# YuvalNirkin/hyperseg

Hardware: AMD Instinct MI355X
Metric: frames/sec @ bs=1 HyperSeg-M 1024x512 (higher is better)
Workload: dtype f32 storage and accumulation; level-4 inverted residual products as 3-term f16 splits (f32-class: 1.3e-7 of sum|a||b|; exact_f32 beside it)

## Files before the change

### hyperseg_amd/_hip.py

```python
import ctypes as C
import os
import types

import torch

_LIB_PATH = os.environ.get('HS_HIP_LIB') or os.path.join(os.path.dirname(os.path.abspath(__file__)), 'lib',
                                                         'libhyperseg_hip.so')

ACT_NONE, ACT_RELU, ACT_RELU6, ACT_SWISH = 0, 1, 2, 3
PAD_MODES = {'zeros': 0, 'reflect': 1, 'replicate': 2, 'circular': 3}
PREV_NONE, PREV_SAME, PREV_BILINEAR = 0, 1, 2

_STATUS = {-1: 'bad argument', -2: 'feature map does not tile into the weight grid (H % fh or W % fw != 0)',
           -3: 'unsupported shape', -4: 'tile does not fit the LDS'}


class HipLibraryError(RuntimeError):
    pass


class StageInputC(C.Structure):
    _fields_ = [('skip', C.c_void_p), ('prev', C.c_void_p),
                ('batch', C.c_int32), ('H', C.c_int32), ('W', C.c_int32),
                ('c_skip', C.c_int32), ('c_prev', C.c_int32),
# ... 167 lines not shown
    'hs_label_resize_batch_coded_fwd': ([vp, i32, i32, i32, i32, vp, vp, vp, i32, i32, i32, vp, i32, i32, i32, vp, i32, vp], STATUS),
    'hs_color_jitter_fwd': ([vp, i32, i32, i32, i32, vp, vp, vp, vp, vp], STATUS),
    'hs_gaussian_blur_fwd': ([vp, i32, i32, i32, i32, vp, vp, vp, vp, vp, vp], STATUS),
    'hs_frame_rotate_fwd': ([vp, i32, i32, i32, i32, vp, i32, i32, C.c_uint32, C.c_uint32, vp, vp, vp], STATUS),
    'hs_label_rotate_fwd': ([vp, i32, i32, i32, i32, vp, i32, i32, i32, i32, vp, i32, vp], STATUS),
    'hs_resize_tables_ragged_fwd': ([vp, i32, i32, i32, i32, i32, i32, i32, vp, vp, vp, vp, vp], STATUS),
    'hs_color_jitter_ragged_fwd': ([vp, i32, i32, i32, i32, vp, vp, vp, vp, vp], STATUS),
    'hs_frame_resize_ragged_fwd': ([vp, i32, i32, i32, i32, vp, vp, vp, vp, i32, i32, i32, vp, vp], STATUS),
    'hs_label_resize_ragged_fwd': ([vp, i32, i32, i32, i32, vp, vp, vp, i32, i32, vp, vp], STATUS),
    'hs_frame_rotate_ragged_fwd': ([vp, i32, i32, i32, i32, vp, vp, vp, i32, i32, C.c_uint32, C.c_uint32, vp, vp, vp], STATUS),
    'hs_label_rotate_ragged_fwd': ([vp, i32, i32, i32, vp, vp, vp, i32, i32, i32, i32, vp, i32, vp], STATUS),
    'hs_mbconv_expand_dw_fwd': ([vp, i32, i32, i32, i32, vp, i32, vp, vp, vp, i32, i32, i32, i32, i32, i32, vp, vp, vp, vp, vp], STATUS),
    'hs_se_gate_fwd': ([vp, i32, i32, i32, C.c_float, vp, vp, i32, vp, vp, vp, vp, vp, i32, vp, vp, vp], STATUS),
    'hs_gemm_split_kp': ([i32], C.c_int),
    'hs_gemm_split_fwd': ([vp, vp, vp, vp, vp, i32, vp, vp, i32, i32, i32, i32, i32, vp], STATUS),
    'hs_gemm_split_conv2x2_fwd': ([vp, vp, vp, vp, i32, vp, vp, i32, i32, i32, i32, i32, i32, vp], STATUS),
    'hs_gemm_split_up2_fwd': ([vp, vp, vp, vp, i32, vp, i32, i32, i32, i32, i32, i32, vp], STATUS),
    'hs_depthwise_route': ([i32] * 11, C.c_int),
    'hs_mbconv_route': ([i32] * 11, C.c_int),
    'hs_stem_dw_route': ([i32] * 9, C.c_int),
    'hs_stem_route': ([i32] * 3, C.c_int),
    'hs_se_gate_route': ([i32] * 5, C.c_int),
    'hs_pointwise_route': ([i32] * 5, C.c_int),
    'hs_pooled_shift_fwd': ([vp, i32, C.c_float, vp, vp, vp, i32, i32, vp], STATUS),
}
EXPORTS = list(SIGNATURES)


def check(status, what):
    if status == 0:
# ... 73 lines not shown
```

### hyperseg_amd/build.py

```python
import os
import shutil
import subprocess
import sys

PKG = os.path.dirname(os.path.abspath(__file__))
REPO = os.path.dirname(PKG)
CSRC = os.path.join(PKG, 'csrc')
LIB_DIR = os.path.join(PKG, 'lib')
LIB_PATH = os.path.join(LIB_DIR, 'libhyperseg_hip.so')
SOURCES = ['hs_weights.hip', 'hs_patch_conv.hip', 'hs_patch_conv_gen.hip', 'hs_patch_conv_k1m.hip', 'hs_k1_chain.hip', 'hs_meta_conv.hip', 'hs_patch_ir.hip', 'hs_patch_ir_fused.hip', 'hs_patch_irc.hip', 'hs_patch_ir_px.hip', 'hs_patch_ir_d2.hip', 'hs_encoder.hip', 'hs_mbconv.hip', 'hs_mbconv_lean.hip', 'hs_gemm_split.hip', 'hs_patch_conv_bwd.hip', 'hs_patch_conv_train.hip', 'hs_train_aux.hip', 'hs_s2w_train.hip', 'hs_eval.hip', 'hs_tta_merge.hip', 'hs_ingest.hip', 'hs_overlay.hip', 'hs_confidence.hip', 'hs_resample.hip', 'hs_resample_batch.hip', 'hs_jitter.hip', 'hs_blur.hip', 'hs_validate.hip', 'hs_rotate.hip', 'hs_augment_ragged.hip', 'hs_label_codec.hip']
HEADERS = [os.path.join(CSRC, 'hs_common.h'), os.path.join(CSRC, 'hs_ir_tiles.h'), os.path.join(CSRC, 'hs_ir_common.h'), os.path.join(CSRC, 'hs_s2w_blocked.h'), os.path.join(CSRC, 'hs_se_tail.h'), os.path.join(CSRC, 'hs_upsample_taps.h'), os.path.join(CSRC, 'hs_ingest.h'), os.path.join(CSRC, 'hs_resample_px.h'), os.path.join(CSRC, 'hs_resample_tables.h'), os.path.join(CSRC, 'hs_jitter_px.h'), os.path.join(CSRC, 'hs_blur_px.h'), os.path.join(CSRC, 'hs_rotate_px.h'), os.path.join(CSRC, 'hs_eval_count.h'), os.path.join(CSRC, 'hs_last_launch.h'), os.path.join(CSRC, 'hs_confidence.h'), os.path.join(CSRC, 'hs_label_codec.h'), os.path.join(REPO, 'include', 'hyperseg_hip.h')]
FLAGS = ['--offload-arch=gfx950', '-O3', '-std=c++17', '-fPIC', '-ffp-contract=off', '-mllvm', '-amdgpu-kernarg-preload-count=16',
         '-Wall', '-Wno-unused-function', '-I', os.path.join(REPO, 'include'), '-I', CSRC]


def _hipcc():
    for cand in (os.environ.get('HIPCC'), shutil.which('hipcc'), '/opt/rocm/bin/hipcc'):
        if cand and os.path.exists(cand):
            return cand
    raise RuntimeError('hipcc not found (need ROCm >= 7.0 with gfx950 support)')


def needs_build():
    if not os.path.exists(LIB_PATH):
        return True
    t = os.path.getmtime(LIB_PATH)
# ... 36 lines not shown
```

### hyperseg_amd/csrc/hs_gemm_split.hip

```cpp
#include "hs_common.h"
#include <type_traits>

namespace hs {

using half8 = __attribute__((ext_vector_type(8))) _Float16;
using gs_f32x4 = __attribute__((ext_vector_type(4))) float;

__device__ __forceinline__ int gs_exp_of(float m) { return min(max(__float_as_int(m) >> 23, 27), 254); }
__device__ __forceinline__ float gs_scale_of(int eb) { return __int_as_float((268 - eb) << 23); }
__device__ __forceinline__ float gs_inv_scale_of(int eb) { return __int_as_float((eb - 14) << 23); }

struct GemmSplitArgs {
    const _Float16* __restrict__ wf;
    const float* __restrict__ w_inv;
    const float* __restrict__ gate; const float* __restrict__ x;
    const float* shift;
    const float* residual;
    float* y;
    int M, K, KST, N, act;
    int conv_wo;
    float* pool_partial;
    int up2_wo;
};

#ifndef HS_GS_NARROW_MAX_WG
#define HS_GS_NARROW_MAX_WG 128
#endif

#ifndef HS_GS_TALL_MIN_WG
#define HS_GS_TALL_MIN_WG 257
#endif

template <int KS, int NWV, bool FAST, int NS, int MT, int NCH, bool PATCH>
__global__ __launch_bounds__(64 * NWV)
void gemm_split_kernel(GemmSplitArgs a) {
    extern __shared__ __attribute__((aligned(16))) float gs_red[];
    constexpr int nthr = 64 * NWV, nwv = NWV;
    constexpr int NP = 16 * NS, NR = 16 * MT, NE = NR * NP;
    const int tid = threadIdx.x, lane = tid & 63, wave = tid >> 6;
    const int lrow = lane & 15, kg = lane >> 4;
    const int n0 = blockIdx.x * NP, r0 = blockIdx.y * MT, b = blockIdx.z;
    const float* __restrict__ xb = a.x + (size_t)b * a.K * a.N;
    const float* __restrict__ gb = a.gate ? a.gate + (size_t)b * a.K : nullptr;
    float* yb = a.y + (size_t)b * a.M * a.N * (a.up2_wo > 0 ? 4 : 1);
    const float* rb = a.residual ? a.residual + (size_t)b * a.M * a.N : nullptr;
    const int rt_max = (a.M + 15) >> 4;

    using gs_f32x2 = __attribute__((ext_vector_type(2))) float;
    const int ncol0 = min(n0 + NS * lrow, a.N - (FAST && !PATCH && NS == 2 ? 2 : 1)), ncol1 = min(n0 + NS * lrow + 1, a.N - 1);
    float xv[NCH][NS][KS][8];
// ... 33 lines not shown
                        const gs_f32x2 v = *reinterpret_cast<const gs_f32x2*>(xb + (size_t)kc * a.N + ncol0);
                        xv[c][0][s][j] = v[0]; xv[c][1][s][j] = v[1];
                    } else {
                        xv[c][0][s][j] = xb[(size_t)kc * a.N + ncol0]; xv[c][1][s][j] = xb[(size_t)kc * a.N + ncol1];
                    }
                }
    }
    constexpr int NG = PATCH ? 1 : NCH;
    float gv[NG][KS][8];
    if constexpr (!PATCH) {
#pragma unroll
        for (int c = 0; c < NCH; ++c)
#pragma unroll
            for (int s = 0; s < KS; ++s) {
                const int k0 = ((wave * NCH + c) * KS + s) * 32 + 8 * kg;
                if constexpr (FAST) {
                    const float* gp = gb ? gb + min(k0, a.K - 8) : a.w_inv;
                    const gs_f32x4 g0 = *reinterpret_cast<const gs_f32x4*>(gp), g1 = *reinterpret_cast<const gs_f32x4*>(gp + 4);
#pragma unroll
                    for (int j = 0; j < 4; ++j) { gv[c][s][j] = g0[j]; gv[c][s][4 + j] = g1[j]; }
                } else {
#pragma unroll
                    for (int j = 0; j < 8; ++j) gv[c][s][j] = gb ? gb[min(k0 + j, a.K - 1)] : 1.0f;
                }
            }
    }
    half8 ah[2][KS], al[2][KS];
    auto load_a = [&](int q) {
        const int rt = min(r0 + q % MT, rt_max - 1);
#pragma unroll
        for (int s = 0; s < KS; ++s) {
// ... 5 lines not shown
    load_a(0);
    constexpr int TE = (NE + nthr - 1) / nthr;
    float wi[TE], sh[TE], yo[TE];
    auto load_tail = [&]() {
#pragma unroll
        for (int i = 0; i < TE; ++i) {
            const int e = min(tid + i * nthr, NE - 1);
            const int row = min(16 * r0 + e / NP, a.M - 1), col = min(n0 + (e & (NP - 1)), a.N - 1);
            wi[i] = a.w_inv[min(16 * r0 + e / NP, 16 * rt_max - 1)];
            sh[i] = a.shift ? a.shift[row] : 0.0f;
            yo[i] = rb ? rb[(size_t)row * a.N + col] : 0.0f;
        }
    };
    constexpr bool LATE_TAIL = KS * NCH >= 3;
    if constexpr (!LATE_TAIL) load_tail();
    __builtin_amdgcn_sched_barrier(0);

    gs_f32x4 tot[MT][NS];
#pragma unroll
    for (int c = 0; c < NCH; ++c) {
        float invb[NS];
        half8 bh[NS][KS], bl[NS][KS];
#pragma unroll
        for (int t = 0; t < NS; ++t) {
            unsigned mx = 0;
#pragma unroll
            for (int s = 0; s < KS; ++s) {
                const int k0 = ((wave * NCH + c) * KS + s) * 32 + 8 * kg;
#pragma unroll
                for (int j = 0; j < 8; ++j) {
                    const float mk = (FAST || PATCH ? k0 : k0 + j) < a.K ? 1.0f : 0.0f;
                    float g = mk;
                    if constexpr (!PATCH) g = gb ? gv[c][s][j] * mk : mk;
                    xv[c][t][s][j] *= g;
                    mx = max(mx, __float_as_uint(xv[c][t][s][j]) & 0x7fffffffu);
                }
            }
            {
                auto r16 = __builtin_amdgcn_permlane16_swap(mx, mx, false, false);
                mx = max(r16[0], r16[1]);
                auto r32 = __builtin_amdgcn_permlane32_swap(mx, mx, false, false);
                mx = max(r32[0], r32[1]);
            }
            const int eb = gs_exp_of(__uint_as_float(mx));
            const float sc = gs_scale_of(eb);
            invb[t] = gs_inv_scale_of(eb);
#pragma unroll
            for (int s = 0; s < KS; ++s) {
// ... 128 lines not shown
    nch = per > 5 ? 2 : 1;
    ks = (steps + nwv * nch - 1) / (nwv * nch);
    return ks <= 5;
}

}

using namespace hs;

extern "C" int hs_gemm_split_kp(int32_t c_in) {
    int nwv, ks, nch;
    if (c_in <= 0 || !gemm_split_plan(c_in, nwv, ks, nch)) return HS_ERR_UNSUPPORTED;
    return nwv * nch * ks * 32;
}

static int launch_gemm_split_plain(const void* w_frag, const float* w_inv, const float* gate, const float* x, const float* shift,
                                   int32_t act, const float* residual, float* y, int32_t batch, int32_t c_out, int32_t c_in,
                                   int32_t kp, int32_t pixels, int up2_wo, void* stream) {
    if (!w_frag || !w_inv || !x || !y || batch <= 0 || c_out <= 0 || c_in <= 0 || pixels <= 0) return HS_ERR_BAD_ARG;
    if (act < 0 || act > 3) return HS_ERR_BAD_ARG;
    int nwv, ks, nch;
    if (!gemm_split_plan(c_in, nwv, ks, nch)) return HS_ERR_UNSUPPORTED;
    if (kp != nwv * nch * ks * 32 || (ks > 1 && nwv != 8)) return HS_ERR_BAD_ARG;
    if (batch > 65535 || (c_out + 31) / 32 > 65535) return HS_ERR_UNSUPPORTED;
    GemmSplitArgs a{(const _Float16*)w_frag, w_inv, gate, x, shift, residual, y, c_out, c_in, kp / 32, pixels, act, 0, nullptr, up2_wo};
    dim3 grid((pixels + 31) / 32, ((c_out + 15) / 16 + 1) / 2, batch);
    const size_t wgs = (size_t)grid.x * grid.y * grid.z;
    const bool narrow = wgs <= HS_GS_NARROW_MAX_WG && pixels > 16;
    const bool tall = wgs >= HS_GS_TALL_MIN_WG && c_out > 32;
    if (narrow) grid.x = (pixels + 15) / 16;
    if (tall) grid.y = ((c_out + 15) / 16 + 3) / 4;
    const size_t lds = (size_t)nwv * (narrow ? 512 : tall ? 2048 : 1024) * sizeof(float);
    hipStream_t s = (hipStream_t)stream;
    const bool fast = (c_in & 7) == 0 && (pixels & 1) == 0 && c_in >= 8;
#define HS_GS_(KSV, NWV, F) do { \
        if (narrow) hipLaunchKernelGGL((gemm_split_kernel<KSV, NWV, F, 1, 2, 1, false>), grid, dim3(64 * NWV), lds, s, a); \
        else if (tall) hipLaunchKernelGGL((gemm_split_kernel<KSV, NWV, F, 2, 4, 1, false>), grid, dim3(64 * NWV), lds, s, a); \
        else hipLaunchKernelGGL((gemm_split_kernel<KSV, NWV, F, 2, 2, 1, false>), grid, dim3(64 * NWV), lds, s, a); } while (0)
#define HS_GS(KSV, NWV) do { if (fast) HS_GS_(KSV, NWV, true); else HS_GS_(KSV, NWV, false); } while (0)
    if (nch == 2) {
        if (!fast || up2_wo > 0) return HS_ERR_UNSUPPORTED;
        grid.x = (pixels + 15) / 16; grid.y = ((c_out + 15) / 16 + 1) / 2;
        const size_t lds2 = (size_t)8 * 512 * sizeof(float);
#define HS_GS2(KSV) hipLaunchKernelGGL((gemm_split_kernel<KSV, 8, true, 1, 2, 2, false>), grid, dim3(512), lds2, s, a)
        switch (ks) { case 3: HS_GS2(3); break; case 4: HS_GS2(4); break; case 5: HS_GS2(5); break; default: return HS_ERR_UNSUPPORTED; }
#undef HS_GS2
        return launch_status();
    }
    switch (ks) {
        case 1: if (nwv == 2) HS_GS(1, 2); else if (nwv == 4) HS_GS(1, 4); else HS_GS(1, 8); break;
        case 2: HS_GS(2, 8); break;
        case 3: HS_GS(3, 8); break;
        case 4: HS_GS(4, 8); break;
        default: HS_GS(5, 8); break;
    }
#undef HS_GS
#undef HS_GS_
    return launch_status();
}

extern "C" int hs_gemm_split_fwd(const void* w_frag, const float* w_inv, const float* gate, const float* x,
                                 const float* shift, int32_t act, const float* residual, float* y,
                                 int32_t batch, int32_t c_out, int32_t c_in, int32_t kp, int32_t pixels, void* stream) {
    return launch_gemm_split_plain(w_frag, w_inv, gate, x, shift, act, residual, y, batch, c_out, c_in, kp, pixels, 0, stream);
}

extern "C" int hs_gemm_split_up2_fwd(const void* w_frag, const float* w_inv, const float* x, const float* shift, int32_t act,
                                     float* y, int32_t batch, int32_t c_out, int32_t c_in, int32_t kp, int32_t Ho, int32_t Wo,
                                     void* stream) {
    if (Ho <= 0 || Wo <= 0 || (((size_t)y) & 7) != 0) return HS_ERR_BAD_ARG;
    return launch_gemm_split_plain(w_frag, w_inv, nullptr, x, shift, act, nullptr, y, batch, c_out, c_in, kp, Ho * Wo, Wo, stream);
}
// ... 10 lines not shown
extern "C" int hs_gemm_split_conv2x2_fwd(const void* w_frag, const float* w_inv, const float* x, const float* shift, int32_t act,
                                         float* y, float* pool_partial, int32_t batch, int32_t c_out, int32_t c_in, int32_t kp,
                                         int32_t Ho, int32_t Wo, void* stream) {
    if (!w_frag || !w_inv || !x || !y || batch <= 0 || c_out <= 0 || c_in <= 0 || Ho <= 0 || Wo <= 0) return HS_ERR_BAD_ARG;
    if (act < 0 || act > 3) return HS_ERR_BAD_ARG;
    int nwv, ks, nch;
    if (c_in > (1 << 20) || !gemm_split_plan(4 * c_in, nwv, ks, nch) || nwv != 8 || (Wo & 1) || (c_in & 1)) return HS_ERR_UNSUPPORTED;
    if (kp != nwv * nch * ks * 32) return HS_ERR_BAD_ARG;
    if ((((size_t)x) & 15) != 0) return HS_ERR_BAD_ARG;
    const int pixels = Ho * Wo;
    if (batch > 65535 || (c_out + 31) / 32 > 65535) return HS_ERR_UNSUPPORTED;
    GemmSplitArgs a{(const _Float16*)w_frag, w_inv, nullptr, x, shift, nullptr, y, c_out, 4 * c_in, kp / 32, pixels, act, Wo, pool_partial, 0};
    dim3 grid((pixels + 15) / 16, ((c_out + 15) / 16 + 1) / 2, batch);
    const size_t lds = (size_t)8 * 512 * sizeof(float);
    hipStream_t s = (hipStream_t)stream;
#define HS_GP(KSV, NCHV) hipLaunchKernelGGL((gemm_split_kernel<KSV, 8, true, 1, 2, NCHV, true>), grid, dim3(512), lds, s, a)
    switch (ks * 2 + nch - 1) {
        case 2: HS_GP(1, 1); break;
        case 4: HS_GP(2, 1); break;
        case 6: HS_GP(3, 1); break;
        case 8: HS_GP(4, 1); break;
        case 10: HS_GP(5, 1); break;
        case 7: HS_GP(3, 2); break;
        case 9: HS_GP(4, 2); break;
        case 11: HS_GP(5, 2); break;
        default: return HS_ERR_UNSUPPORTED;
    }
#undef HS_GP
    return launch_status();
}
```

### hyperseg_amd/functional.py

```python
import collections
import ctypes as C
import functools
import os
import threading

import torch

from . import _hip
from ._hip import ACT_NONE, ACT_RELU, ACT_RELU6, PAD_MODES

BN_EPS_DEFAULT = 1e-5
DTYPE_CODES = {torch.float32: 0, torch.bfloat16: 1, torch.float16: 2}
S2W_TRAIN_MAX_LAYERS = 8
COSCHEDULE_BANKS = os.environ.get('HS_COSCHEDULE_BANKS', '0') == '1'


def _round_up(n, m):
    return (n + m - 1) // m * m


def _device_of(a):
    if isinstance(a, torch.Tensor):
        return a.device
    if isinstance(a, (StageInput, BankRef, SignalRef, U8Frame)):
# ... 1097 lines not shown
        raise ValueError(f'out has shape {tuple(out.shape)}, expected {shape}')
    if residual is not None and tuple(residual.shape) != shape:
        raise ValueError(f'residual has shape {tuple(residual.shape)}, expected {shape}')
    if gate is not None and tuple(gate.shape) != (b, cin):
        raise ValueError(f'gate has shape {tuple(gate.shape)}, expected {(b, cin)}')
    if shift is not None and shift.numel() != sw.c_out:
        raise ValueError(f'shift has {shift.numel()} entries, expected {sw.c_out}')
    _hip.run.hs_gemm_split_fwd(_hip.dev_ptr(sw.frag, 'w_frag', torch.float16), _hip.dev_ptr(sw.inv, 'w_inv'),
                               _hip.dev_ptr(gate, 'gate') if gate is not None else None, _hip.dev_ptr(x, 'x'),
                               _hip.dev_ptr(shift, 'shift') if shift is not None else None, int(act),
                               _hip.dev_ptr(residual, 'residual') if residual is not None else None,
                               _hip.dev_ptr(out, 'out'), b, sw.c_out, cin, sw.kp, h * w, _hip.stream_ptr())
    return out


@_on_operand_device
def gemm_split_conv2x2(sw, x, shift=None, act=ACT_NONE, out=None, pool_partial=None):
    b, cin, h, w = x.shape
    if 4 * cin != sw.c_in:
        raise ValueError(f'input has {cin} channels, the weight {sw.c_in} / 4')
    if h % 2 or w % 4:
        raise ValueError(f'map {h}x{w}: height must be even and width a multiple of 4')
    shape = (b, sw.c_out, h // 2, w // 2)
    if out is None:
        out = torch.empty(shape, device=x.device, dtype=torch.float32)
    elif tuple(out.shape) != shape:
        raise ValueError(f'out has shape {tuple(out.shape)}, expected {shape}')
    if shift is not None and shift.numel() != sw.c_out:
        raise ValueError(f'shift has {shift.numel()} entries, expected {sw.c_out}')
    nblk = -(-(h // 2) * (w // 2) // 16)
# ... 1018 lines not shown
```

### hyperseg_amd/utils/inference.py

```python
import contextlib
import os

import torch
import torch.nn as nn

from ..models._common import Blend, Epilogue, HyperGenBase, Score


class InputNorm:

    LAYOUTS = ('hwc', 'chw')

    def __init__(self, mean=(0.485, 0.456, 0.406), std=(0.229, 0.224, 0.225), layout='hwc'):
        if layout not in self.LAYOUTS:
            raise ValueError(f'layout {layout!r}: expected one of {self.LAYOUTS}')
        self.mean = torch.as_tensor(mean, dtype=torch.float32).flatten().clone()
        self.std = torch.as_tensor(std, dtype=torch.float32).flatten().clone()
        if self.mean.numel() != 3 or self.std.numel() != 3:
            raise ValueError('mean and std must hold one value per channel of a 3-channel frame')
        if bool((self.std == 0).any()):
            raise ValueError('std must be non-zero')
        self.layout = layout
        values = torch.arange(256, dtype=torch.float32)
        self._tables = {torch.device('cpu'): ((values.div(255)[None, :] - self.mean[:, None]) / self.std[:, None]).contiguous()}
# ... 179 lines not shown
            _fold(mods[i], mods[i + 1])
            seq[i + 1] = nn.Identity()
            n += 1
    return n


def _bn_affine(bn):
    with torch.no_grad():
        scale = bn.weight / torch.sqrt(bn.running_var + bn.eps)
        shift = bn.bias - bn.running_mean * scale
    return scale.detach().clone(), shift.detach().clone()


SPLIT_GEMM_MAX_K = int(os.environ.get('HS_SPLIT_GEMM_MAX_K', '1280'))
STEM_DW = os.environ.get('HS_STEM_DW', '1') != '0'
FUSE_EXPAND_MIN_PIXELS = int(os.environ.get('HS_FUSE_EXPAND_MIN_PIXELS', '2048'))
FUSE_EXPAND_MAX_CIN = int(os.environ.get('HS_FUSE_EXPAND_MAX_CIN', '40'))


LEAN_MFMA_MAX_CIN = int(os.environ.get('HS_LEAN_MFMA_MAX_CIN', '16'))
PW_MFMA_MAX_CIN = int(os.environ.get('HS_PW_MFMA_MAX_CIN', '96'))
PW_MFMA_MIN_PIXELS = int(os.environ.get('HS_PW_MFMA_MIN_PIXELS', '8192'))
GEMM_LT_MIN_PIXELS = int(os.environ.get('HS_GEMM_LT_MIN_PIXELS', '16384'))


@contextlib.contextmanager
def gemm_library(pixels, batch=1):
    want = os.environ.get('HS_BLAS') or ('cublaslt' if (pixels >= GEMM_LT_MIN_PIXELS or batch > 1) else 'cublas')
    prev = torch.backends.cuda.preferred_blas_library()
    torch.backends.cuda.preferred_blas_library(want)
# ... 185 lines not shown
                else:
                    x = self.expand(x)
            out = HF.depthwise_conv_bn_act(x, blk._depthwise_conv.weight, self.stride, self.pad_t, self.pad_l,
                                           (ho, wo), self.scale, self.shift, act=3, pool=True,
                                           in_scale=in_scale, in_shift=in_shift, se=se)
        y, pooled, gated = out if se is not None else (out[0], out[1], False)

        def se_gate(**fold):
            if gated and not fold:
                return pooled
            return HF.se_gate(pooled, b, ho * wo, red.weight, red.bias, self._exp_t, exp.bias, **fold)
        skip = inputs.contiguous() if self.skip else None
        if lean_gemm:
            sw = proj.split_weights(True, y.device) if proj.split_gemm else None
            if sw is not None:
                gate = se_gate()
                if self.defer_shift:
                    if skip is None:
                        return HF.gemm_split(sw, y, gate=gate)
                    return HF.gemm_split(sw, y, gate=gate, residual=skip, out=skip)
                return HF.gemm_split(sw, y, gate=gate, shift=proj.shift, residual=skip)
            wp = se_gate(w_proj=proj.conv.weight, out_scale=proj.scale)
            cmid = y.shape[1]
            with gemm_library(ho * wo, b):
                if b == 1:
                    w2d, y2d = wp.view(-1, cmid), y.view(cmid, ho * wo)
                    if self.defer_shift:
                        if skip is None:
                            return torch.mm(w2d, y2d).view(1, -1, ho, wo)
                        skip.view(-1, ho * wo).addmm_(w2d, y2d)
# ... 480 lines not shown
```

### include/hyperseg_hip.h

```cpp
#ifndef HYPERSEG_HIP_H
#define HYPERSEG_HIP_H

#include <stdint.h>

#ifdef __cplusplus
extern "C" {
#endif

#define HS_ABI_VERSION 1

typedef enum {
    HS_OK = 0,
    HS_ERR_BAD_ARG = -1,
    HS_ERR_NOT_DIVISIBLE = -2,
    HS_ERR_UNSUPPORTED = -3,
    HS_ERR_LDS = -4
} hs_status;

typedef enum { HS_ACT_NONE = 0, HS_ACT_RELU = 1, HS_ACT_RELU6 = 2, HS_ACT_SWISH = 3 } hs_act;
typedef enum { HS_PAD_ZEROS = 0, HS_PAD_REFLECT = 1, HS_PAD_REPLICATE = 2, HS_PAD_CIRCULAR = 3 } hs_pad_mode;
typedef enum { HS_PREV_NONE = 0, HS_PREV_SAME = 1, HS_PREV_BILINEAR = 2 } hs_prev_mode;

typedef struct {
    const float* skip;
// ... 360 lines not shown
                    int32_t Ho, int32_t Wo, int32_t aligned16, int32_t with_se_tail);
int hs_stem_dw_route(int32_t H, int32_t W, int32_t c_mid, int32_t stem_pad_t, int32_t stem_pad_l, int32_t Hs, int32_t Ws,
                     int32_t k, int32_t aligned16);
#define HS_SE_ROUTE_FUSED 0
#define HS_SE_ROUTE_EARLY 1
#define HS_SE_ROUTE_FUSED_WIDE 2
#define HS_SE_ROUTE_TWO_LAUNCH 3
int hs_se_gate_route(int32_t channels, int32_t nblk, int32_t c_squeezed, int32_t with_w_proj, int32_t aligned16);
#define HS_PW_ROUTE(nb, nt, vec) (((nb) << 8) | ((nt) << 4) | (vec))
int hs_pointwise_route(int32_t batch, int32_t c_in, int32_t c_out, int32_t pixels, int32_t aligned16);

int hs_gemm_split_kp(int32_t c_in);
int hs_gemm_split_fwd(const void* w_frag, const float* w_inv, const float* gate, const float* x, const float* shift,
                      int32_t act, const float* residual, float* y, int32_t batch, int32_t c_out, int32_t c_in, int32_t kp,
                      int32_t pixels, void* stream);
int hs_gemm_split_conv2x2_fwd(const void* w_frag, const float* w_inv, const float* x, const float* shift, int32_t act, float* y,
                              float* pool_partial, int32_t batch, int32_t c_out, int32_t c_in, int32_t kp, int32_t Ho,
                              int32_t Wo, void* stream);
int hs_gemm_split_up2_fwd(const void* w_frag, const float* w_inv, const float* x, const float* shift, int32_t act, float* y,
                          int32_t batch, int32_t c_out, int32_t c_in, int32_t kp, int32_t Ho, int32_t Wo, void* stream);
int hs_pooled_shift_fwd(const float* partial, int32_t nblk, float inv_pixels, const float* wb, const float* shift,
                        float* shift_out, int32_t rows, int32_t channels, void* stream);

int hs_halo_tiles_fwd(int32_t dtype, const void* x, int32_t batch, int32_t channels, int32_t H, int32_t W, int32_t fh, int32_t fw,
                      void* tiled, int32_t patch_major, void* stream);
int hs_halo_tiles_bwd(int32_t dtype, const void* dtiled, int32_t batch, int32_t channels, int32_t H, int32_t W, int32_t fh, int32_t fw,
                      void* dx, int32_t patch_major, void* stream);
int hs_tile_interior_fwd(int32_t dtype, const void* tiled, int32_t batch, int32_t channels, int32_t H, int32_t W, int32_t fh,
                         int32_t fw, void* y, void* stream);
int hs_tile_interior_bwd(int32_t dtype, const void* dy, int32_t batch, int32_t channels, int32_t H, int32_t W, int32_t fh, int32_t fw,
// ... 112 lines not shown
```

Measured before the change: 1357.

## Fuse SE gate computation into split-GEMM projection kernel prologue

```diff
diff --git a/hyperseg_amd/_hip.py b/hyperseg_amd/_hip.py
--- a/hyperseg_amd/_hip.py
+++ b/hyperseg_amd/_hip.py
@@ -205,6 +205,8 @@
     'hs_se_gate_fwd': ([vp, i32, i32, i32, C.c_float, vp, vp, i32, vp, vp, vp, vp, vp, i32, vp, vp, vp], STATUS),
     'hs_gemm_split_kp': ([i32], C.c_int),
     'hs_gemm_split_fwd': ([vp, vp, vp, vp, vp, i32, vp, vp, i32, i32, i32, i32, i32, vp], STATUS),
+    'hs_gemm_split_se_fwd': ([vp, vp, vp, i32, C.c_float, vp, vp, i32, vp, vp, vp, vp, i32, vp, vp, i32, i32, i32, i32, i32, vp, vp, vp], STATUS),
+    'hs_gemm_split_se_route': ([i32] * 6, C.c_int),
     'hs_gemm_split_conv2x2_fwd': ([vp, vp, vp, vp, i32, vp, vp, i32, i32, i32, i32, i32, i32, vp], STATUS),
     'hs_gemm_split_up2_fwd': ([vp, vp, vp, vp, i32, vp, i32, i32, i32, i32, i32, i32, vp], STATUS),
     'hs_depthwise_route': ([i32] * 11, C.c_int),
diff --git a/hyperseg_amd/build.py b/hyperseg_amd/build.py
--- a/hyperseg_amd/build.py
+++ b/hyperseg_amd/build.py
@@ -9,7 +9,7 @@
 LIB_DIR = os.path.join(PKG, 'lib')
 LIB_PATH = os.path.join(LIB_DIR, 'libhyperseg_hip.so')
 SOURCES = ['hs_weights.hip', 'hs_patch_conv.hip', 'hs_patch_conv_gen.hip', 'hs_patch_conv_k1m.hip', 'hs_k1_chain.hip', 'hs_meta_conv.hip', 'hs_patch_ir.hip', 'hs_patch_ir_fused.hip', 'hs_patch_irc.hip', 'hs_patch_ir_px.hip', 'hs_patch_ir_d2.hip', 'hs_encoder.hip', 'hs_mbconv.hip', 'hs_mbconv_lean.hip', 'hs_gemm_split.hip', 'hs_patch_conv_bwd.hip', 'hs_patch_conv_train.hip', 'hs_train_aux.hip', 'hs_s2w_train.hip', 'hs_eval.hip', 'hs_tta_merge.hip', 'hs_ingest.hip', 'hs_overlay.hip', 'hs_confidence.hip', 'hs_resample.hip', 'hs_resample_batch.hip', 'hs_jitter.hip', 'hs_blur.hip', 'hs_validate.hip', 'hs_rotate.hip', 'hs_augment_ragged.hip', 'hs_label_codec.hip']
-HEADERS = [os.path.join(CSRC, 'hs_common.h'), os.path.join(CSRC, 'hs_ir_tiles.h'), os.path.join(CSRC, 'hs_ir_common.h'), os.path.join(CSRC, 'hs_s2w_blocked.h'), os.path.join(CSRC, 'hs_se_tail.h'), os.path.join(CSRC, 'hs_upsample_taps.h'), os.path.join(CSRC, 'hs_ingest.h'), os.path.join(CSRC, 'hs_resample_px.h'), os.path.join(CSRC, 'hs_resample_tables.h'), os.path.join(CSRC, 'hs_jitter_px.h'), os.path.join(CSRC, 'hs_blur_px.h'), os.path.join(CSRC, 'hs_rotate_px.h'), os.path.join(CSRC, 'hs_eval_count.h'), os.path.join(CSRC, 'hs_last_launch.h'), os.path.join(CSRC, 'hs_confidence.h'), os.path.join(CSRC, 'hs_label_codec.h'), os.path.join(REPO, 'include', 'hyperseg_hip.h')]
+HEADERS = [os.path.join(CSRC, 'hs_common.h'), os.path.join(CSRC, 'hs_ir_tiles.h'), os.path.join(CSRC, 'hs_ir_common.h'), os.path.join(CSRC, 'hs_s2w_blocked.h'), os.path.join(CSRC, 'hs_se_tail.h'), os.path.join(CSRC, 'hs_se_gate_phases.h'), os.path.join(CSRC, 'hs_upsample_taps.h'), os.path.join(CSRC, 'hs_ingest.h'), os.path.join(CSRC, 'hs_resample_px.h'), os.path.join(CSRC, 'hs_resample_tables.h'), os.path.join(CSRC, 'hs_jitter_px.h'), os.path.join(CSRC, 'hs_blur_px.h'), os.path.join(CSRC, 'hs_rotate_px.h'), os.path.join(CSRC, 'hs_eval_count.h'), os.path.join(CSRC, 'hs_last_launch.h'), os.path.join(CSRC, 'hs_confidence.h'), os.path.join(CSRC, 'hs_label_codec.h'), os.path.join(REPO, 'include', 'hyperseg_hip.h')]
 FLAGS = ['--offload-arch=gfx950', '-O3', '-std=c++17', '-fPIC', '-ffp-contract=off', '-mllvm', '-amdgpu-kernarg-preload-count=16',
          '-Wall', '-Wno-unused-function', '-I', os.path.join(REPO, 'include'), '-I', CSRC]
 
diff --git a/hyperseg_amd/csrc/hs_gemm_split.hip b/hyperseg_amd/csrc/hs_gemm_split.hip
--- a/hyperseg_amd/csrc/hs_gemm_split.hip
+++ b/hyperseg_amd/csrc/hs_gemm_split.hip
@@ -1,4 +1,5 @@
 #include "hs_common.h"
+#include "hs_se_gate_phases.h"
 #include <type_traits>
 
 namespace hs {
@@ -23,6 +24,16 @@
     int up2_wo;
 };
 
+struct GemmSeArgs {
+    const float* __restrict__ partial;
+    const float* __restrict__ w1; const float* __restrict__ b1;
+    const float* __restrict__ w2t; const float* __restrict__ b2;
+    float* gate_out; float* squeezed_out;
+    float inv_hw; int nblk, Csq;
+};
+template <bool SEG> struct GemmSeOperand {};
+template <> struct GemmSeOperand<true> : GemmSeArgs {};
+
 #ifndef HS_GS_NARROW_MAX_WG
 #define HS_GS_NARROW_MAX_WG 128
 #endif
@@ -31,9 +42,10 @@
 #define HS_GS_TALL_MIN_WG 257
 #endif
 
-template <int KS, int NWV, bool FAST, int NS, int MT, int NCH, bool PATCH>
+template <int KS, int NWV, bool FAST, int NS, int MT, int NCH, bool PATCH, bool SEG = false>
 __global__ __launch_bounds__(64 * NWV)
-void gemm_split_kernel(GemmSplitArgs a) {
+void gemm_split_kernel(GemmSplitArgs a, GemmSeOperand<SEG> se) {
+    static_assert(!SEG || (FAST && !PATCH && NCH == 1 && (NWV == 8 ? KS <= 3 : KS == 1)), "SEG: the project convolutions' forms only");
     extern __shared__ __attribute__((aligned(16))) float gs_red[];
     constexpr int nthr = 64 * NWV, nwv = NWV;
     constexpr int NP = 16 * NS, NR = 16 * MT, NE = NR * NP;
@@ -97,7 +109,8 @@
 #pragma unroll
             for (int s = 0; s < KS; ++s) {
                 const int k0 = ((wave * NCH + c) * KS + s) * 32 + 8 * kg;
-                if constexpr (FAST) {
+                if constexpr (SEG) {
+                } else if constexpr (FAST) {
                     const float* gp = gb ? gb + min(k0, a.K - 8) : a.w_inv;
                     const gs_f32x4 g0 = *reinterpret_cast<const gs_f32x4*>(gp), g1 = *reinterpret_cast<const gs_f32x4*>(gp + 4);
 #pragma unroll
@@ -133,7 +146,43 @@
     };
     constexpr bool LATE_TAIL = KS * NCH >= 3;
     if constexpr (!LATE_TAIL) load_tail();
+    constexpr int SE_PV = SEP_MAX_UNITS / nthr, SE_RW = SEP_MAX_CSQ / NWV, SE_W1U = NWV == 8 ? (KS < 3 ? KS : 3) : 1;
+    constexpr int SE_CI = NWV == 8 && KS >= 3 ? 2 : 1;
+    float4 se_pv[SE_PV], se_w1v[SE_RW][SE_W1U];
+    float se_b1v[SE_RW], se_w2q[SE_CI][4][8], se_b2v[SE_CI];
+    if constexpr (SEG) {
+        se_load_units<nthr, SE_PV>(se.partial + (size_t)b * a.K * se.nblk, se.nblk, a.K, tid, se_pv);
+        se_load_reduce<NWV, SE_RW, SE_W1U>(se.w1, se.b1, a.K, se.Csq, wave, lane, se_w1v, se_b1v);
+#pragma unroll
+        for (int ci = 0; ci < SE_CI; ++ci) se_load_expand(se.w2t, se.b2, a.K, se.Csq, min(tid + nthr * ci, a.K - 1), se_w2q[ci], se_b2v[ci]);
+    }
     __builtin_amdgcn_sched_barrier(0);
+    if constexpr (SEG) {
+        float* mean_c = gs_red + SEP_MEAN; float* zs = gs_red + SEP_ZS; float* gate_s = gs_red + SEP_GATE;
+        se_channel_means<nthr, SE_PV>(se_pv, se.nblk, a.K, se.inv_hw, tid, gs_red + SEP_PART, mean_c);
+        se_squeeze_rows<NWV, SE_RW, SE_W1U>(se_w1v, se_b1v, mean_c, a.K, se.Csq, wave, lane, zs);
+        __syncthreads();
+        const bool first = blockIdx.x == 0 && blockIdx.y == 0;
+        if (first && se.squeezed_out && tid < se.Csq) se.squeezed_out[(size_t)b * se.Csq + tid] = zs[tid];
+#pragma unroll
+        for (int ci = 0; ci < SE_CI; ++ci) {
+            const int ch = tid + nthr * ci;
+            const float g = se_channel_gate(se_w2q[ci], se_b2v[ci], zs, se.Csq);
+            if (ch < a.K) {
+                gate_s[ch] = g;
+                if (first && se.gate_out) se.gate_out[(size_t)b * a.K + ch] = g;
+            }
+        }
+        __syncthreads();
+#pragma unroll
+        for (int s = 0; s < KS; ++s) {
+            const float* gp = gate_s + min((wave * KS + s) * 32 + 8 * kg, a.K - 8);
+            const gs_f32x4 g0 = *reinterpret_cast<const gs_f32x4*>(gp), g1 = *reinterpret_cast<const gs_f32x4*>(gp + 4);
+#pragma unroll
+            for (int j = 0; j < 4; ++j) { gv[0][s][j] = g0[j]; gv[0][s][4 + j] = g1[j]; }
+        }
+        __syncthreads();
+    }
 
     gs_f32x4 tot[MT][NS];
 #pragma unroll
@@ -150,7 +199,7 @@
                 for (int j = 0; j < 8; ++j) {
                     const float mk = (FAST || PATCH ? k0 : k0 + j) < a.K ? 1.0f : 0.0f;
                     float g = mk;
-                    if constexpr (!PATCH) g = gb ? gv[c][s][j] * mk : mk;
+                    if constexpr (!PATCH) g = SEG || gb ? gv[c][s][j] * mk : mk;
                     xv[c][t][s][j] *= g;
                     mx = max(mx, __float_as_uint(xv[c][t][s][j]) & 0x7fffffffu);
                 }
@@ -309,35 +358,51 @@
     return nwv * nch * ks * 32;
 }
 
+struct GemmSplitPolicy {
+    int nwv, ks, nch;
+    bool narrow, tall, fast;
+    dim3 grid;
+    size_t lds;
+};
+static int gemm_split_policy(int batch, int c_out, int c_in, int kp, int pixels, GemmSplitPolicy& p) {
+    if (!gemm_split_plan(c_in, p.nwv, p.ks, p.nch)) return HS_ERR_UNSUPPORTED;
+    if (kp != p.nwv * p.nch * p.ks * 32 || (p.ks > 1 && p.nwv != 8)) return HS_ERR_BAD_ARG;
+    if (batch > 65535 || (c_out + 31) / 32 > 65535) return HS_ERR_UNSUPPORTED;
+    p.grid = dim3((pixels + 31) / 32, ((c_out + 15) / 16 + 1) / 2, batch);
+    const size_t wgs = (size_t)p.grid.x * p.grid.y * p.grid.z;
+    p.narrow = wgs <= HS_GS_NARROW_MAX_WG && pixels > 16;
+    p.tall = wgs >= HS_GS_TALL_MIN_WG && c_out > 32;
+    if (p.narrow) p.grid.x = (pixels + 15) / 16;
+    if (p.tall) p.grid.y = ((c_out + 15) / 16 + 3) / 4;
+    p.lds = (size_t)p.nwv * (p.narrow ? 512 : p.tall ? 2048 : 1024) * sizeof(float);
+    p.fast = (c_in & 7) == 0 && (pixels & 1) == 0 && c_in >= 8;
+    return HS_OK;
+}
+
 static int launch_gemm_split_plain(const void* w_frag, const float* w_inv, const float* gate, const float* x, const float* shift,
                                    int32_t act, const float* residual, float* y, int32_t batch, int32_t c_out, int32_t c_in,
                                    int32_t kp, int32_t pixels, int up2_wo, void* stream) {
     if (!w_frag || !w_inv || !x || !y || batch <= 0 || c_out <= 0 || c_in <= 0 || pixels <= 0) return HS_ERR_BAD_ARG;
     if (act < 0 || act > 3) return HS_ERR_BAD_ARG;
-    int nwv, ks, nch;
-    if (!gemm_split_plan(c_in, nwv, ks, nch)) return HS_ERR_UNSUPPORTED;
-    if (kp != nwv * nch * ks * 32 || (ks > 1 && nwv != 8)) return HS_ERR_BAD_ARG;
-    if (batch > 65535 || (c_out + 31) / 32 > 65535) return HS_ERR_UNSUPPORTED;
+    GemmSplitPolicy pol;
+    const int pst = gemm_split_policy(batch, c_out, c_in, kp, pixels, pol);
+    if (pst != HS_OK) return pst;
+    const int nwv = pol.nwv, ks = pol.ks, nch = pol.nch;
+    const bool narrow = pol.narrow, tall = pol.tall, fast = pol.fast;
+    dim3 grid = pol.grid;
+    const size_t lds = pol.lds;
     GemmSplitArgs a{(const _Float16*)w_frag, w_inv, gate, x, shift, residual, y, c_out, c_in, kp / 32, pixels, act, 0, nullptr, up2_wo};
-    dim3 grid((pixels + 31) / 32, ((c_out + 15) / 16 + 1) / 2, batch);
-    const size_t wgs = (size_t)grid.x * grid.y * grid.z;
-    const bool narrow = wgs <= HS_GS_NARROW_MAX_WG && pixels > 16;
-    const bool tall = wgs >= HS_GS_TALL_MIN_WG && c_out > 32;
-    if (narrow) grid.x = (pixels + 15) / 16;
-    if (tall) grid.y = ((c_out + 15) / 16 + 3) / 4;
-    const size_t lds = (size_t)nwv * (narrow ? 512 : tall ? 2048 : 1024) * sizeof(float);
     hipStream_t s = (hipStream_t)stream;
-    const bool fast = (c_in & 7) == 0 && (pixels & 1) == 0 && c_in >= 8;
 #define HS_GS_(KSV, NWV, F) do { \
-        if (narrow) hipLaunchKernelGGL((gemm_split_kernel<KSV, NWV, F, 1, 2, 1, false>), grid, dim3(64 * NWV), lds, s, a); \
-        else if (tall) hipLaunchKernelGGL((gemm_split_kernel<KSV, NWV, F, 2, 4, 1, false>), grid, dim3(64 * NWV), lds, s, a); \
-        else hipLaunchKernelGGL((gemm_split_kernel<KSV, NWV, F, 2, 2, 1, false>), grid, dim3(64 * NWV), lds, s, a); } while (0)
+        if (narrow) hipLaunchKernelGGL((gemm_split_kernel<KSV, NWV, F, 1, 2, 1, false>), grid, dim3(64 * NWV), lds, s, a, GemmSeOperand<false>{}); \
+        else if (tall) hipLaunchKernelGGL((gemm_split_kernel<KSV, NWV, F, 2, 4, 1, false>), grid, dim3(64 * NWV), lds, s, a, GemmSeOperand<false>{}); \
+        else hipLaunchKernelGGL((gemm_split_kernel<KSV, NWV, F, 2, 2, 1, false>), grid, dim3(64 * NWV), lds, s, a, GemmSeOperand<false>{}); } while (0)
 #define HS_GS(KSV, NWV) do { if (fast) HS_GS_(KSV, NWV, true); else HS_GS_(KSV, NWV, false); } while (0)
     if (nch == 2) {
         if (!fast || up2_wo > 0) return HS_ERR_UNSUPPORTED;
         grid.x = (pixels + 15) / 16; grid.y = ((c_out + 15) / 16 + 1) / 2;
         const size_t lds2 = (size_t)8 * 512 * sizeof(float);
-#define HS_GS2(KSV) hipLaunchKernelGGL((gemm_split_kernel<KSV, 8, true, 1, 2, 2, false>), grid, dim3(512), lds2, s, a)
+#define HS_GS2(KSV) hipLaunchKernelGGL((gemm_split_kernel<KSV, 8, true, 1, 2, 2, false>), grid, dim3(512), lds2, s, a, GemmSeOperand<false>{})
         switch (ks) { case 3: HS_GS2(3); break; case 4: HS_GS2(4); break; case 5: HS_GS2(5); break; default: return HS_ERR_UNSUPPORTED; }
 #undef HS_GS2
         return launch_status();
@@ -351,6 +416,54 @@
     }
 #undef HS_GS
 #undef HS_GS_
+    return launch_status();
+}
+
+static int gemm_split_se_route(int channels, int nblk, int c_squeezed, int c_out, int pixels, bool aligned16, int batch, GemmSplitPolicy& pol) {
+    if (channels <= 0 || nblk <= 0 || c_squeezed <= 0 || c_out <= 0 || pixels <= 0 || batch <= 0) return HS_ERR_BAD_ARG;
+    const int kp = hs_gemm_split_kp(channels);
+    if (kp < 0) return HS_ERR_UNSUPPORTED;
+    const int pst = gemm_split_policy(batch, c_out, channels, kp, pixels, pol);
+    if (pst != HS_OK) return pst;
+    if (hs_se_gate_route(channels, nblk, c_squeezed, 0, aligned16 ? 1 : 0) != HS_SE_ROUTE_FUSED) return HS_ERR_UNSUPPORTED;
+    if (!aligned16 || !pol.fast || pol.nch != 1 || channels > SEP_MAX_C || c_squeezed > SEP_MAX_CSQ) return HS_ERR_UNSUPPORTED;
+    if (pol.ks > (pol.nwv == 8 ? 3 : 1)) return HS_ERR_UNSUPPORTED;
+    return HS_GSE_ROUTE(pol.ks, pol.nwv);
+}
+
+extern "C" int hs_gemm_split_se_route(int32_t channels, int32_t nblk, int32_t c_squeezed, int32_t c_out, int32_t pixels, int32_t aligned16) {
+    GemmSplitPolicy pol;
+    return gemm_split_se_route(channels, nblk, c_squeezed, c_out, pixels, aligned16 != 0, 1, pol);
+}
+
+extern "C" int hs_gemm_split_se_fwd(const void* w_frag, const float* w_inv, const float* partial, int32_t nblk, float inv_hw,
+                                    const float* w_reduce, const float* b_reduce, int32_t c_squeezed, const float* w_expand_t,
+                                    const float* b_expand, const float* x, const float* shift, int32_t act, const float* residual,
+                                    float* y, int32_t batch, int32_t c_out, int32_t c_in, int32_t kp, int32_t pixels,
+                                    float* gate_out, float* squeezed_out, void* stream) {
+    if (!w_frag || !w_inv || !x || !y || batch <= 0 || c_out <= 0 || c_in <= 0 || pixels <= 0) return HS_ERR_BAD_ARG;
+    if (!partial || !w_reduce || !b_reduce || !w_expand_t || !b_expand || nblk <= 0 || c_squeezed <= 0) return HS_ERR_BAD_ARG;
+    if (act < 0 || act > 3) return HS_ERR_BAD_ARG;
+    GemmSplitPolicy pol;
+    const bool aligned16 = (((size_t)partial | (size_t)w_reduce) & 15) == 0;
+    const int route = gemm_split_se_route(c_in, nblk, c_squeezed, c_out, pixels, aligned16, batch, pol);
+    if (route < 0) return route;
+    if (kp != pol.nwv * pol.ks * 32) return HS_ERR_BAD_ARG;
+    GemmSplitArgs a{(const _Float16*)w_frag, w_inv, nullptr, x, shift, residual, y, c_out, c_in, kp / 32, pixels, act, 0, nullptr, 0};
+    GemmSeOperand<true> se{{partial, w_reduce, b_reduce, w_expand_t, b_expand, gate_out, squeezed_out, inv_hw, nblk, c_squeezed}};
+    const size_t se_lds = (size_t)SEP_LDS_FLOATS * sizeof(float);
+    const size_t lds = pol.lds > se_lds ? pol.lds : se_lds;
+    hipStream_t s = (hipStream_t)stream;
+#define HS_GSE(KSV, NWV) do { \
+        if (pol.narrow) hipLaunchKernelGGL((gemm_split_kernel<KSV, NWV, true, 1, 2, 1, false, true>), pol.grid, dim3(64 * NWV), lds, s, a, se); \
+        else if (pol.tall) hipLaunchKernelGGL((gemm_split_kernel<KSV, NWV, true, 2, 4, 1, false, true>), pol.grid, dim3(64 * NWV), lds, s, a, se); \
+        else hipLaunchKernelGGL((gemm_split_kernel<KSV, NWV, true, 2, 2, 1, false, true>), pol.grid, dim3(64 * NWV), lds, s, a, se); } while (0)
+    switch (pol.ks) {
+        case 1: if (pol.nwv == 2) HS_GSE(1, 2); else if (pol.nwv == 4) HS_GSE(1, 4); else HS_GSE(1, 8); break;
+        case 2: HS_GSE(2, 8); break;
+        default: HS_GSE(3, 8); break;
+    }
+#undef HS_GSE
     return launch_status();
 }
 
@@ -391,7 +504,7 @@
     dim3 grid((pixels + 15) / 16, ((c_out + 15) / 16 + 1) / 2, batch);
     const size_t lds = (size_t)8 * 512 * sizeof(float);
     hipStream_t s = (hipStream_t)stream;
-#define HS_GP(KSV, NCHV) hipLaunchKernelGGL((gemm_split_kernel<KSV, 8, true, 1, 2, NCHV, true>), grid, dim3(512), lds, s, a)
+#define HS_GP(KSV, NCHV) hipLaunchKernelGGL((gemm_split_kernel<KSV, 8, true, 1, 2, NCHV, true>), grid, dim3(512), lds, s, a, GemmSeOperand<false>{})
     switch (ks * 2 + nch - 1) {
         case 2: HS_GP(1, 1); break;
         case 4: HS_GP(2, 1); break;
diff --git a/hyperseg_amd/csrc/hs_se_gate_phases.h b/hyperseg_amd/csrc/hs_se_gate_phases.h
--- /dev/null
+++ b/hyperseg_amd/csrc/hs_se_gate_phases.h
@@ -0,0 +1,113 @@
+#pragma once
+#include "hs_common.h"
+
+namespace hs {
+
+constexpr int SEP_MAX_C = 768, SEP_MAX_CSQ = 32, SEP_MAX_UNITS = 2048;
+constexpr int SEP_MEAN = 0, SEP_ZS = SEP_MEAN + SEP_MAX_C, SEP_GATE = SEP_ZS + SEP_MAX_CSQ, SEP_PART = SEP_GATE + SEP_MAX_C;
+constexpr int SEP_LDS_FLOATS = SEP_PART + SEP_MAX_UNITS + SEP_MAX_C;
+
+template <int NTHR, int PV>
+__device__ __forceinline__ void se_load_units(const float* __restrict__ pb, int nblk, int C, int tid, float4 (&pv)[PV]) {
+    const bool vec = (nblk & 3) == 0;
+    const int units = C * (vec ? nblk >> 2 : nblk);
+    if (vec) {
+#pragma unroll
+        for (int k = 0; k < PV; ++k) pv[k] = reinterpret_cast<const float4*>(pb)[min(tid + NTHR * k, units - 1)];
+    } else {
+#pragma unroll
+        for (int k = 0; k < PV; ++k) pv[k] = make_float4(pb[min(tid + NTHR * k, units - 1)], 0.0f, 0.0f, 0.0f);
+    }
+}
+
+template <int NTHR, int PV>
+__device__ __forceinline__ void se_channel_means(const float4 (&pv)[PV], int nblk, int C, float inv_hw, int tid, float* part, float* mean) {
+    const int qn = (nblk & 3) == 0 ? nblk >> 2 : nblk, units = C * qn;
+#pragma unroll
+    for (int k = 0; k < PV; ++k) {
+        const int e = tid + NTHR * k;
+        if (e < units) {
+            const int ch = e / qn;
+            part[ch * (qn + 1) + (e - ch * qn)] = (pv[k].x + pv[k].y) + (pv[k].z + pv[k].w);
+        }
+    }
+    __syncthreads();
+    for (int ch = tid; ch < C; ch += NTHR) {
+        const float* run = part + ch * (qn + 1);
+        float t = 0.0f;
+        for (int i = 0; i < qn; ++i) t += run[i];
+        mean[ch] = t * inv_hw;
+    }
+    __syncthreads();
+}
+
+template <int NWV, int RW, int W1U>
+__device__ __forceinline__ void se_load_reduce(const float* __restrict__ w1, const float* __restrict__ b1, int C, int Csq, int wave, int lane,
+                                               float4 (&w1v)[RW][W1U], float (&b1v)[RW]) {
+    const int c4 = C >> 2;
+#pragma unroll
+    for (int r = 0; r < RW; ++r) {
+        const int j = min(wave + NWV * r, Csq - 1);
+        b1v[r] = b1[j];
+#pragma unroll
+        for (int u = 0; u < W1U; ++u) {
+            w1v[r][u] = make_float4(0.0f, 0.0f, 0.0f, 0.0f);
+            if (NWV * r < Csq && 64 * u < c4)
+                w1v[r][u] = reinterpret_cast<const float4*>(w1 + (size_t)j * C)[min(lane + 64 * u, c4 - 1)];
+        }
+    }
+}
+
+template <int NWV, int RW, int W1U>
+__device__ __forceinline__ void se_squeeze_rows(const float4 (&w1v)[RW][W1U], const float (&b1v)[RW], const float* mean, int C, int Csq,
+                                                int wave, int lane, float* zs) {
+    const int c4 = C >> 2;
+    float4 mv[W1U];
+#pragma unroll
+    for (int u = 0; u < W1U; ++u) {
+        const int k = lane + 64 * u;
+        mv[u] = *reinterpret_cast<const float4*>(mean + 4 * min(k, c4 - 1));
+        if (k >= c4) mv[u] = make_float4(0.0f, 0.0f, 0.0f, 0.0f);
+    }
+#pragma unroll
+    for (int r = 0; r < RW; ++r) {
+        if (NWV * r < Csq) {
+            float a = 0.0f;
+#pragma unroll
+            for (int u = 0; u < W1U; ++u) {
+                a = fmaf(w1v[r][u].x, mv[u].x, a); a = fmaf(w1v[r][u].y, mv[u].y, a);
+                a = fmaf(w1v[r][u].z, mv[u].z, a); a = fmaf(w1v[r][u].w, mv[u].w, a);
+            }
+            a = wave_sum64(a);
+            const int j = wave + NWV * r;
+            if (lane == 0 && j < Csq) zs[j] = swishf(a + b1v[r]);
+        }
+    }
+}
+
+__device__ __forceinline__ void se_load_expand(const float* __restrict__ w2t, const float* __restrict__ b2, int C, int Csq, int c,
+                                               float (&w2q)[4][8], float& b2v) {
+    const int jq = (Csq + 3) >> 2;
+#pragma unroll
+    for (int i = 0; i < 4; ++i)
+#pragma unroll
+        for (int u = 0; u < 8; ++u) w2q[i][u] = w2t[(size_t)min(i * jq + u, Csq - 1) * C + c];
+    b2v = b2[c];
+}
+
+__device__ __forceinline__ float se_channel_gate(const float (&w2q)[4][8], float b2v, const float* zs, int Csq) {
+    const int jq = (Csq + 3) >> 2;
+    float q[4];
+#pragma unroll
+    for (int i = 0; i < 4; ++i) {
+        const int j0 = i * jq, j1 = min(j0 + jq, Csq);
+        float acc = 0.0f;
+#pragma unroll
+        for (int u = 0; u < 8; ++u)
+            if (j0 + u < j1) acc = fmaf(w2q[i][u], zs[min(j0 + u, SEP_MAX_CSQ - 1)], acc);
+        q[i] = acc;
+    }
+    return sigmoidf_fast(((q[0] + q[1]) + (q[2] + q[3])) + b2v);
+}
+
+}
diff --git a/hyperseg_amd/functional.py b/hyperseg_amd/functional.py
--- a/hyperseg_amd/functional.py
+++ b/hyperseg_amd/functional.py
@@ -1135,6 +1135,49 @@
     return out
 
 
+def gemm_split_se_route(channels, nblk, c_squeezed, c_out, pixels, aligned=True):
+    r = _route(_hip.lib.hs_gemm_split_se_route(channels, nblk, c_squeezed, c_out, pixels, int(bool(aligned))), 'hs_gemm_split_se_route')
+    return None if r is None else f'ks{r >> 4}_w{r & 15}'
+
+
+@_on_operand_device
+def gemm_split_se(sw, x, partial, hw, w_reduce, b_reduce, w_expand_t, b_expand, shift=None, act=ACT_NONE, residual=None, out=None,
+                  gate_out=None, squeezed_out=None):
+    b, cin, h, w = x.shape
+    if cin != sw.c_in:
+        raise ValueError(f'input has {cin} channels, the weight {sw.c_in}')
+    shape = (b, sw.c_out, h, w)
+    if out is None:
+        out = torch.empty(shape, device=x.device, dtype=torch.float32)
+    elif tuple(out.shape) != shape:
+        raise ValueError(f'out has shape {tuple(out.shape)}, expected {shape}')
+    if residual is not None and tuple(residual.shape) != shape:
+        raise ValueError(f'residual has shape {tuple(residual.shape)}, expected {shape}')
+    if shift is not None and shift.numel() != sw.c_out:
+        raise ValueError(f'shift has {shift.numel()} entries, expected {sw.c_out}')
+    if partial.dim() != 2 or partial.shape[0] != b * cin:
+        raise ValueError(f'partial has shape {tuple(partial.shape)}, expected ({b * cin}, nblk)')
+    csq = w_reduce.shape[0]
+    if w_reduce.numel() != csq * cin or b_reduce.numel() != csq:
+        raise ValueError(f'w_reduce / b_reduce have {w_reduce.numel()} / {b_reduce.numel()} entries, expected {csq * cin} / {csq}')
+    if tuple(w_expand_t.shape) != (csq, cin) or b_expand.numel() != cin:
+        raise ValueError(f'w_expand_t has shape {tuple(w_expand_t.shape)} and b_expand {b_expand.numel()} entries, expected {(csq, cin)} and {cin}')
+    if gate_out is not None and tuple(gate_out.shape) != (b, cin):
+        raise ValueError(f'gate_out has shape {tuple(gate_out.shape)}, expected {(b, cin)}')
+    if squeezed_out is not None and tuple(squeezed_out.shape) != (b, csq):
+        raise ValueError(f'squeezed_out has shape {tuple(squeezed_out.shape)}, expected {(b, csq)}')
+    _hip.run.hs_gemm_split_se_fwd(_hip.dev_ptr(sw.frag, 'w_frag', torch.float16), _hip.dev_ptr(sw.inv, 'w_inv'),
+                                  _hip.dev_ptr(partial, 'partial'), partial.shape[1], 1.0 / float(hw),
+                                  _hip.dev_ptr(w_reduce, 'w_reduce'), _hip.dev_ptr(b_reduce, 'b_reduce'), csq,
+                                  _hip.dev_ptr(w_expand_t, 'w_expand_t'), _hip.dev_ptr(b_expand, 'b_expand'), _hip.dev_ptr(x, 'x'),
+                                  _hip.dev_ptr(shift, 'shift') if shift is not None else None, int(act),
+                                  _hip.dev_ptr(residual, 'residual') if residual is not None else None,
+                                  _hip.dev_ptr(out, 'out'), b, sw.c_out, cin, sw.kp, h * w,
+                                  _hip.dev_ptr(gate_out, 'gate_out') if gate_out is not None else None,
+                                  _hip.dev_ptr(squeezed_out, 'squeezed_out') if squeezed_out is not None else None, _hip.stream_ptr())
+    return out
+
+
 @_on_operand_device
 def gemm_split_conv2x2(sw, x, shift=None, act=ACT_NONE, out=None, pool_partial=None):
     b, cin, h, w = x.shape
diff --git a/hyperseg_amd/utils/inference.py b/hyperseg_amd/utils/inference.py
--- a/hyperseg_amd/utils/inference.py
+++ b/hyperseg_amd/utils/inference.py
@@ -217,6 +217,8 @@
 
 SPLIT_GEMM_MAX_K = int(os.environ.get('HS_SPLIT_GEMM_MAX_K', '1280'))
 STEM_DW = os.environ.get('HS_STEM_DW', '1') != '0'
+HS_GEMM_SE = os.environ.get('HS_GEMM_SE', '1') != '0'
+GEMM_SE_MAX_CIN = 512
 FUSE_EXPAND_MIN_PIXELS = int(os.environ.get('HS_FUSE_EXPAND_MIN_PIXELS', '2048'))
 FUSE_EXPAND_MAX_CIN = int(os.environ.get('HS_FUSE_EXPAND_MAX_CIN', '40'))
 
@@ -432,6 +434,15 @@
         if lean_gemm:
             sw = proj.split_weights(True, y.device) if proj.split_gemm else None
             if sw is not None:
+                if (HS_GEMM_SE and y.is_cuda and not gated and cmid <= GEMM_SE_MAX_CIN and
+                        HF.gemm_split_se_route(cmid, pooled.shape[1], self._red_w.shape[0], sw.c_out, ho * wo,
+                                               aligned=(pooled.data_ptr() | red.weight.data_ptr()) % 16 == 0) is not None):
+                    se_ops = (pooled, ho * wo, red.weight, red.bias, self._exp_t, exp.bias)
+                    if self.defer_shift:
+                        if skip is None:
+                            return HF.gemm_split_se(sw, y, *se_ops)
+                        return HF.gemm_split_se(sw, y, *se_ops, residual=skip, out=skip)
+                    return HF.gemm_split_se(sw, y, *se_ops, shift=proj.shift, residual=skip)
                 gate = se_gate()
                 if self.defer_shift:
                     if skip is None:
diff --git a/include/hyperseg_hip.h b/include/hyperseg_hip.h
--- a/include/hyperseg_hip.h
+++ b/include/hyperseg_hip.h
@@ -398,6 +398,13 @@
 int hs_gemm_split_fwd(const void* w_frag, const float* w_inv, const float* gate, const float* x, const float* shift,
                       int32_t act, const float* residual, float* y, int32_t batch, int32_t c_out, int32_t c_in, int32_t kp,
                       int32_t pixels, void* stream);
+#define HS_GSE_ROUTE(ks, nwv) (((ks) << 4) | (nwv))
+int hs_gemm_split_se_fwd(const void* w_frag, const float* w_inv, const float* partial, int32_t nblk, float inv_hw,
+                         const float* w_reduce, const float* b_reduce, int32_t c_squeezed, const float* w_expand_t,
+                         const float* b_expand, const float* x, const float* shift, int32_t act, const float* residual,
+                         float* y, int32_t batch, int32_t c_out, int32_t c_in, int32_t kp, int32_t pixels,
+                         float* gate_out, float* squeezed_out, void* stream);
+int hs_gemm_split_se_route(int32_t channels, int32_t nblk, int32_t c_squeezed, int32_t c_out, int32_t pixels, int32_t aligned16);
 int hs_gemm_split_conv2x2_fwd(const void* w_frag, const float* w_inv, const float* x, const float* shift, int32_t act, float* y,
                               float* pool_partial, int32_t batch, int32_t c_out, int32_t c_in, int32_t kp, int32_t Ho,
                               int32_t Wo, void* stream);
```

New measurement: 1378 (median of 6 runs). 1.02x the previous value.
